# tan9zj/xnrs

Measured on AMD Instinct MI355X. Metric: impressions/sec (encode+score) on MIND-shaped batches, higher is better.
Workload: dtype f32; 1 GPU; NRMS full user+news encode + 5-candidate dot scoring (BASELINE configs[2]; token shape of config/mind_small_NRMS.yml); batch_impressions_per_gpu=512, history=50, candidates=5, d_backbone=768, n_heads=16, emb_dim=256, parallelism=impressions sharded by user over 1 GPU(s), no data-path collective

## Files before the change

### xnrs_amd/csrc/batch.hip

```cpp
#include <atomic>

#include "host.h"

namespace xnrs {

__device__ __forceinline__ uint64_t mix64(uint64_t seed, uint64_t a, uint64_t b) {
  uint64_t z = seed + 0x9E3779B97F4A7C15ull * (a * 0x100000001B3ull + b + 1);
  z = (z ^ (z >> 30)) * 0xBF58476D1CE4E5B9ull;
  z = (z ^ (z >> 27)) * 0x94D049BB133111EBull;
  return z ^ (z >> 31);
}

__global__ __launch_bounds__(256) void assemble_train_kernel(BatchArgs a) {
  const int64_t i = (int64_t)blockIdx.x * 256 + threadIdx.x;
  const int W = a.l_hist + 1 + a.n_neg;
  if (i >= a.B * W) return;
  const int64_t b = i / W;
  const int j = (int)(i - b * W);
  const int64_t s = a.sess[b];
  if (j < a.l_hist) {
    const int64_t lo = a.hist_off[s], hi = a.hist_off[s + 1];
    const int64_t n = (hi - lo < a.l_hist) ? (hi - lo) : a.l_hist;
    a.hist_out[b * a.l_hist + j] = (j < n) ? a.hist_val[hi - n + j] : a.pad_row;
  } else {
// ... 260 lines not shown
        w += __popcll(b);
        if (kept && sl < S) kv_src[e1 + sl] = (int32_t)(src0 + sl);
      }
      if (lane == 0) kv_block[j] = e1 / S;
    }
    __syncthreads();
  }
  bad = __syncthreads_or(bad);
  if (tid == 0) {
    counts[0] = s_carry[0];
    counts[1] = s_carry[1];
    counts[2] = bad ? 1 : 0;
  }
}

__global__ __launch_bounds__(1024) void compact_rows64_kernel(const float* __restrict__ mask, const int32_t* __restrict__ ids,
                                                               int64_t n_news, int64_t chunk, int S, int64_t* __restrict__ row_off_all,
                                                               int32_t* __restrict__ live_all, int32_t* __restrict__ kvs_all,
                                                               int32_t* __restrict__ kvb_all, int64_t* __restrict__ counts_all) {
  __shared__ unsigned long long s_bits[1024];
  __shared__ int64_t s_row[1024];
  __shared__ int s_ex[2][1024];
  __shared__ int s_wsum[2][16];
  __shared__ int s_carry[2];
  const int tid = threadIdx.x, wave = tid >> 6, lane = tid & 63;
  const int64_t news0 = (int64_t)blockIdx.x * chunk;
  const int cn = (int)(n_news - news0 < chunk ? n_news - news0 : chunk);
  int64_t* row_off = row_off_all + (int64_t)blockIdx.x * (chunk + 1);
  int32_t* live_src = live_all + (int64_t)blockIdx.x * chunk * S;
  int32_t* kv_src = kvs_all + (int64_t)blockIdx.x * chunk * S;
  int32_t* kv_block = kvb_all + (int64_t)blockIdx.x * chunk;
  int64_t* counts = counts_all + 3 * (int64_t)blockIdx.x;
  int bad = 0;
  if (tid < 2) s_carry[tid] = 0;
  if (tid == 0) row_off[0] = 0;
  for (int base = 0; base < cn; base += 1024) {
    const int nn = cn - base < 1024 ? cn - base : 1024;
    s_bits[tid] = 0ull;
    s_row[tid] = tid < nn ? (ids ? (int64_t)ids[news0 + base + tid] : news0 + base + tid) : 0;
    __syncthreads();
    const int n_el = nn * S;
    for (int i0 = tid; i0 < n_el; i0 += 4096) {
      float mv[4];
      int jj[4], sl[4];
#pragma unroll
      for (int u = 0; u < 4; ++u) {
        const int i = i0 + 1024 * u;
        jj[u] = (i < n_el ? i : 0) / S;
        sl[u] = (i < n_el ? i : 0) - jj[u] * S;
        mv[u] = i < n_el ? mask[s_row[jj[u]] * S + sl[u]] : 0.f;
// ... 13 lines not shown
      int x = v[which];
      for (int off = 1; off < 64; off <<= 1) {
        const int up = __shfl_up(x, off);
        if (lane >= off) x += up;
      }
      incl[which] = x;
      if (lane == 63) s_wsum[which][wave] = x;
    }
    __syncthreads();
    for (int which = 0; which < 2; ++which) {
      int before = s_carry[which];
      for (int w = 0; w < wave; ++w) before += s_wsum[which][w];
      s_ex[which][tid] = before + incl[which] - v[which];
    }
    if (tid < nn) {
      row_off[base + tid + 1] = s_ex[0][tid] + cnt;
      kv_block[base + tid] = s_ex[1][tid] / S;
    }
    __syncthreads();
    if (tid == 1023) {
      s_carry[0] = s_ex[0][1023] + v[0];
      s_carry[1] = s_ex[1][1023] + v[1];
    }
#pragma unroll 4
    for (int i = tid; i < n_el; i += 1024) {
      const int jj = i / S, sl = i - jj * S;
      const unsigned long long b = s_bits[jj];
      if (b == 0ull) continue;
      const int32_t src = (int32_t)(s_row[jj] * S + sl);
      kv_src[s_ex[1][jj] + sl] = src;
      if ((b >> sl) & 1ull) live_src[s_ex[0][jj] + __popcll(b & ((1ull << sl) - 1ull))] = src;
    }
    __syncthreads();
  }
  bad = __syncthreads_or(bad);
  if (tid == 0) {
    counts[0] = s_carry[0];
    counts[1] = s_carry[1];
    counts[2] = bad ? 1 : 0;
  }
}

__global__ __launch_bounds__(256) void row_counts_kernel(const float* __restrict__ mask, const int32_t* __restrict__ ids,
                                                          int64_t n_seq, int L, int32_t* __restrict__ cnt) {
  const int lane = threadIdx.x & 63;
  const int64_t seq = (int64_t)blockIdx.x * 4 + (threadIdx.x >> 6);
  if (seq >= n_seq) return;
  const float* mp = mask + (ids ? (int64_t)ids[seq] : seq) * L;
// ... 126 lines not shown
  return w;
}
void set_status_word(int32_t* w) {
  int dev = -1;
  (void)hipGetDevice(&dev);
  g_status_device.store(w ? dev : -1, std::memory_order_relaxed);
  g_status_word.store(w, std::memory_order_relaxed);
}

hipError_t launch_compact_rows(const float* mask, const int32_t* ids, int64_t n_news, int64_t chunk, int S, int64_t* row_off,
                               int32_t* live_src, int32_t* kv_src, int32_t* kv_block, int64_t* counts, hipStream_t stream) {
  if (n_news <= 0 || chunk <= 0) return hipSuccess;
  const int64_t passes = (n_news + chunk - 1) / chunk;
  if (passes > 0x7fffffffLL) return hipErrorInvalidValue;
  if (S <= 64)
    hipLaunchKernelGGL(compact_rows64_kernel, dim3((unsigned)passes), dim3(1024), 0, stream, mask, ids, n_news, chunk, S, row_off,
                       live_src, kv_src, kv_block, counts);
  else
    hipLaunchKernelGGL(compact_rows_kernel, dim3((unsigned)passes), dim3(1024), 0, stream, mask, ids, n_news, chunk, S, row_off,
                       live_src, kv_src, kv_block, counts);
  return hipGetLastError();
}

__global__ __launch_bounds__(1024) void live_tiles_kernel(const float* __restrict__ mask, const int32_t* __restrict__ ids,
                                                           int64_t n_seq, int64_t chunk, int L, int BM, int64_t cap,
                                                           uint8_t* __restrict__ alive_all, int64_t* __restrict__ n_tiles,
                                                           int32_t* __restrict__ tiles_all) {
  __shared__ int s_wsum[16];
  __shared__ int s_carry;
  const int tid = threadIdx.x, wave = tid >> 6, lane = tid & 63;
  const int64_t seq0 = (int64_t)blockIdx.x * chunk;
  const int64_t cn = n_seq - seq0 < chunk ? n_seq - seq0 : chunk;
  uint8_t* alive = alive_all + seq0;
  int32_t* tiles = tiles_all + (int64_t)blockIdx.x * cap;
  for (int64_t j = tid; j < cn; j += 1024) {
    const float* mp = mask + (ids ? (int64_t)ids[seq0 + j] : seq0 + j) * L;
    int any = 0;
#pragma unroll 4
    for (int s = 0; s < L; ++s) any |= mp[s] != 0.f ? 1 : 0;
    alive[j] = (uint8_t)any;
  }
  if (tid == 0) s_carry = 0;
  __syncthreads();
  const int64_t rows = cn * L;
  const int64_t nt = (rows + BM - 1) / BM;
  const uint64_t below = lane ? (~0ull >> (64 - lane)) : 0ull;
  for (int64_t base = 0; base < nt; base += 1024) {
    const int64_t t = base + tid;
    bool live = false;
    if (t < nt) {
      const int64_t r0 = t * BM, r1 = (r0 + BM < rows ? r0 + BM : rows) - 1;
      for (int64_t n = r0 / L; n <= r1 / L; ++n) live = live || alive[n] != 0;
    }
    const uint64_t b = __ballot(live);
    if (lane == 0) s_wsum[wave] = __popcll(b);
    __syncthreads();
    int before = s_carry;
    for (int w = 0; w < wave; ++w) before += s_wsum[w];
    if (live) tiles[before + __popcll(b & below)] = (int32_t)t;
    __syncthreads();
    if (tid == 0) {
      int tot = s_carry;
      for (int w = 0; w < 16; ++w) tot += s_wsum[w];
      s_carry = tot;
    }
    __syncthreads();
  }
  if (tid == 0) n_tiles[blockIdx.x] = s_carry;
}

hipError_t launch_live_tiles(const float* mask, const int32_t* ids, int64_t n_seq, int64_t chunk, int L, int BM, uint8_t* alive,
                             int64_t* n_tiles, int32_t* tiles, hipStream_t stream) {
  if (n_seq <= 0 || chunk <= 0 || L <= 0 || BM <= 0) return hipSuccess;
  const int64_t passes = (n_seq + chunk - 1) / chunk;
  const int64_t cap = live_tiles_cap(chunk, L, BM);
  if (passes > 0x7fffffffLL || cap > 0x7fffffffLL) return hipErrorInvalidValue;
  hipLaunchKernelGGL(live_tiles_kernel, dim3((unsigned)passes), dim3(1024), 0, stream, mask, ids, n_seq, chunk, L, BM, cap, alive,
                     n_tiles, tiles);
  return hipGetLastError();
}

}

using namespace xnrs;

extern "C" {

size_t xnrs_row_lists_workspace_bytes(int64_t n_seq) { return n_seq > 0 ? align_up((size_t)n_seq * sizeof(int32_t)) : 0; }

int32_t xnrs_build_row_lists(const float* m, const int32_t* ids, int64_t n_seq, int32_t L, int32_t* live_rows,
                             int32_t* live_src_rows, int32_t* kv_rows, int32_t* kv_src_rows, int64_t* counts, void* ws,
                             size_t ws_bytes, void* stream) {
  if (n_seq < 0 || L <= 0 || !m || !live_rows || !kv_rows || !counts) return XNRS_EINVAL;
// ... 60 lines not shown
```

### xnrs_amd/csrc/encoder_fwd.hip

```cpp
#include <vector>

#include "host.h"

using namespace xnrs;

namespace xnrs {

Plan make_plan(int64_t n_seq, int L, int D, int A, int E, bool att, bool additive, bool head, bool pooled, int64_t chunk,
               bool train, int n_heads) {
  Plan p{};
  if (train) chunk = n_seq > 0 ? n_seq : 1;
  if (chunk <= 0) chunk = 65536 / L;
  if (chunk > n_seq) chunk = n_seq;
  if (chunk < 1) chunk = 1;
  p.chunk = chunk;
  const size_t rows = (size_t)chunk * L;
  Carver c;
  p.off_qkv = c.take_if(att, rows * 3 * (size_t)D * F32);
  p.off_o = c.take_if(att, rows * (size_t)D * F32);
  p.off_y = c.take_if(att && pooled, rows * (size_t)D * F32);
  p.off_t = c.take_if(pooled && additive, rows * (size_t)A * F32);
  p.off_p = c.take_if(pooled && head, (size_t)n_seq * D * F32);
  p.off_h = c.take_if(pooled && head, (size_t)n_seq * E * F32);
  p.off_stats = c.take_if(train && att, (size_t)chunk * n_heads * L * 2 * F32);
// ... 3 lines not shown
  if (pooled && additive) pl += align_up(split_planes_bytes(A, D));
  p.off_planes = c.take(pl);
  NewsFusedPlan nf{};
  size_t nfb = 0;
  if (att && additive && !train) {
    if (n_heads <= 0) nfb = news_fused_img_bound_bytes(L, D, A);
    else if (news_fused_plan(L, D, n_heads, A, &nf)) nfb = nf.img_bytes;
  }
  p.off_nf = c.take_if(nfb != 0, nfb);
  p.off_nfo = c.take_if(nfb != 0, news_fused_scratch_bytes(L, D));
  const bool lt = att && pooled && !train;
  const size_t passes = (size_t)(((n_seq > 0 ? n_seq : 1) + chunk - 1) / chunk);
  p.off_lt_alive = c.take_if(lt, (size_t)(n_seq > 0 ? n_seq : 1));
  p.off_lt_n = c.take_if(lt, passes * sizeof(int64_t));
  p.off_lt_tiles = c.take_if(lt, passes * (size_t)live_tiles_cap(chunk, L, LIVE_TILE_BM) * sizeof(int32_t));
  p.fold = carve_fold(c, att && additive, n_seq, D, A);
  p.total = c.total();
  return p;
}

bool device_counts_ok(const float* x, int D, int A, const xnrs_mha_params* att, const xnrs_additive_params* pool) {
  auto al16 = [](const void* p) { return p == nullptr || (reinterpret_cast<uintptr_t>(p) & 15) == 0; };
  if (!knobs().gemm_buf || gemm_mode() != 0 || D % 4 != 0 || D < 4 || (A > 0 && A % 4 != 0)) return false;
  if (!al16(x) || (pool && !al16(pool->w1))) return false;
  if (att && !(al16(att->wq) && al16(att->wk) && al16(att->wv) && al16(att->wo))) return false;
  return (int64_t)D * D * 4 <= (1ll << 30) && (int64_t)A * D * 4 <= (1ll << 30);
}

}

// ... 282 lines not shown
  const bool lt = r.live_tiles && knobs().gemm_live_tiles && !train && pooled && m && att && !fused && !afused &&
                  n_seq * (int64_t)L >= knobs().gemm_live_tiles_min_rows &&
                  device_counts_ok(x, D, A, att, additive ? pool : nullptr);
  bool lt_qkv = false;
  if (lt && knobs().mha_skip_masked) {
    MhaCoreArgs probe = mha_core_args(qkv + D, 3 * (int64_t)D, att, o, p.chunk, L, D);
    probe.q = qkv;
    probe.mask = m;
    probe.skip_dead = 1;
    lt_qkv = mha_core_skips_dead(probe);
  }
  const bool lt_fc1 = lt && additive && rowdot;
  const int64_t lt_cap = live_tiles_cap(p.chunk, L, LIVE_TILE_BM);
  const int64_t* lt_n = at<int64_t>(w, p.off_lt_n);
  const int32_t* lt_tiles = at<int32_t>(w, p.off_lt_tiles);
  if (lt_qkv || lt_fc1)
    XNRS_TRY(launch_live_tiles(m, ids, n_seq, p.chunk, L, LIVE_TILE_BM, at<uint8_t>(w, p.off_lt_alive), at<int64_t>(w, p.off_lt_n),
                               at<int32_t>(w, p.off_lt_tiles), stream));
  std::vector<int64_t> lt_host;
  if ((lt_qkv && prof_on(0)) || (lt_fc1 && prof_on(3))) {
    lt_host.resize((size_t)((n_seq + p.chunk - 1) / p.chunk));
    if (hipStreamSynchronize(stream) != hipSuccess ||
        hipMemcpy(lt_host.data(), lt_n, lt_host.size() * sizeof(int64_t), hipMemcpyDeviceToHost) != hipSuccess)
      lt_host.clear();
  }
  for (int64_t c0 = 0; !fused && !afused && c0 < n_seq; c0 += p.chunk) {
    const int64_t nc = (n_seq - c0 < p.chunk) ? (n_seq - c0) : p.chunk;
    const int64_t rows = nc * L;
    const int64_t* ltn = lt_n + c0 / p.chunk;
    const int32_t* ltl = lt_tiles + (c0 / p.chunk) * lt_cap;
    const double lt_rows = (double)LIVE_TILE_BM *
                           (double)(lt_host.empty() ? (rows + LIVE_TILE_BM - 1) / LIVE_TILE_BM : lt_host[(size_t)(c0 / p.chunk)]);
    const int32_t* cids = ids ? ids + c0 : nullptr;
    const float* cx = ids ? x : x + c0 * (int64_t)L * D;
    const float* cm = m ? (ids ? m : m + c0 * (int64_t)L) : nullptr;

    const float* seq = cx;
    const int32_t* seq_ids = cids;
    if (att) {
      const int64_t ld3 = 3 * (int64_t)D;
      if (qkv_given) {
      } else if (live) {
        const double nl = (double)prof_count(0, cnt, 0, n_live, stream), nkv = (double)prof_count(0, cnt, 1, n_kv, stream);
        ProfScope ps(0, 2.0 * (kvl ? nkv : rows) * 2.0 * D * D + 2.0 * nl * (double)D * D, stream);
        GemmArgs g = qkv_projection(cx, {cids, L}, att, 1, qkv + D, ld3, rows, D, pqkv);
        if (kvl) {
          XNRS_TRY(launch_zero_dead_qkv(qkv, cm, cids, nc, L, D, stream));
// ... 5 lines not shown
          g.m_dev = cnt ? cnt + 1 : nullptr;
          g.m_fill_hint = 0.6f;
          if (n_kv > 0) XNRS_TRY(launch_gemm_f32(g, stream));
        } else {
          XNRS_TRY(launch_gemm_f32(g, stream));
          XNRS_TRY(launch_zero_cols(qkv, ld3, D, rows, stream));
        }
        if (n_live > 0) {
          GemmArgs q = gemm_linear(cx, {lvx, 1}, D, att->wq, att->bq, qkv, ld3, n_live, D, D, XNRS_ACT_NONE, pqkv[0]);
          q.c_scatter = 1;
          q.c_scatter_ids = live_rows;
          q.m_dev = cnt;
          q.m_fill_hint = 0.4f;
          XNRS_TRY(launch_gemm_f32(q, stream));
        }
      } else {
        GemmArgs g = qkv_projection(cx, {cids, L}, att, 0, qkv, ld3, rows, D, pqkv);
        if (lt_qkv) {
          g.live_n = ltn;
          g.live_tiles = ltl;
        }
        ProfScope ps(0, 2.0 * (lt_qkv ? lt_rows : (double)rows) * 3.0 * D * D, stream);
        XNRS_TRY(launch_gemm_f32(g, stream));
      }

      MhaCoreArgs ma = mha_core_args(qkv + D, ld3, att, o, nc, L, D);
      ma.q = qkv;
      ma.mask = cm;
      ma.mask_gather_ids = cids;
      ma.dropout_p = att->dropout_p;
// ... 31 lines not shown

    float* pooled_dst = (head ? pb : y) + c0 * (int64_t)D;
    float* hm_dst = hm ? hm + c0 : nullptr;
    if (additive) {
      if (live) {
        ProfScope ps(3, 2.0 * (double)prof_count(3, cnt, 0, n_live, stream) * (double)D * A, stream);
        XNRS_TRY(hipMemsetAsync(t, 0, (size_t)rows * A * sizeof(float), stream));
        if (n_live > 0) {
          GemmArgs fg = fc1_product(seq, {att ? live_rows : lvx, 1}, fc1, t, n_live, D, A, false, pool, p1);
          fg.c_scatter = 1;
          fg.c_scatter_ids = live_rows;
          fg.m_dev = cnt;
          fg.m_fill_hint = 0.4f;
          XNRS_TRY(launch_gemm_f32(fg, stream));
        }
      } else {
        GemmArgs fg = fc1_product(seq, {seq_ids, L}, fc1, t, rows, D, A, rowdot, pool, p1);
        if (lt_fc1) {
          fg.live_n = ltn;
          fg.live_tiles = ltl;
        }
        ProfScope ps(3, 2.0 * (lt_fc1 ? lt_rows : (double)rows) * (double)D * A, stream);
        XNRS_TRY(launch_gemm_f32(fg, stream));
      }
      AdditivePoolArgs pa = additive_pool_args(t, rowdot, pool, seq, nc, L, D, A);
      pa.skip_dead = lt_fc1 ? 1 : 0;
      pa.mask = cm;
      pa.mask_gather_ids = cids;
      pa.x_gather_ids = seq_ids;
      pa.y = fold ? pob + c0 * (int64_t)D : pooled_dst;
      pa.asum_out = fold ? asum + c0 : nullptr;
      pa.a_out = a_save ? a_save : (a_out ? a_out + c0 * (int64_t)L : nullptr);
      pa.hm_out = cm ? hm_dst : nullptr;
      {
        ProfScope ps(4, 2.0 * rows * (double)(A + D), stream);
        XNRS_TRY(launch_additive_pool(pa, stream));
      }
      if (a_save && a_out)
        XNRS_TRY(hipMemcpyAsync(a_out, a_save, (size_t)rows * sizeof(float), hipMemcpyDeviceToDevice, stream));
    } else {
      MeanPoolArgs mp{};
// ... 342 lines not shown
```

### xnrs_amd/csrc/gemm_f32.hip

```cpp
#include <atomic>
#include <cstdlib>
#include <type_traits>

#include "kernels.h"

namespace xnrs {

constexpr int KALIGN = 32;

__device__ __attribute__((aligned(16))) float g_zero_line[4] = {0.f, 0.f, 0.f, 0.f};

typedef unsigned u32x4 __attribute__((ext_vector_type(4)));
constexpr unsigned BUF_OOB = 0x40000000u;

template <int TM, int TN, bool A_COL, bool B_KN, bool VEC, int PIPE, int BK, bool BUF = false, int MINW = 2, bool GATH = false,
          int KG = 2, bool RDOT = false, bool MDEV = false, bool LIVE = false>
__global__ __launch_bounds__(256, MINW) void gemm_f32_kernel(const GemmArgs a, int m_tiles, int n_tiles_seg, int gn) {
  static_assert(!MDEV || (!A_COL && !B_KN), "device row counts: forward layout only");
  static_assert(!LIVE || (BUF && !MDEV), "live row tiles: buffer-load forward kernels, host row count");
  static_assert(!BUF || (!A_COL && !B_KN && VEC), "buffer loads are implemented for the forward layout");
  static_assert(!RDOT || PIPE == 5, "the fused row dots ride on the interleaved pipeline (its MFMA call is the swapped one)");
  static_assert(!GATH || BUF, "the gathered-A variant keeps buffer loads for B");
  constexpr int BM = 64 * TM, BN = 64 * TN;
  constexpr bool SWZ = BK == 16;
// ... 428 lines not shown
    static_assert(sizeof(float2) * BN <= sizeof(float) * A_SZ * NBUF, "bias / weight staging fits the A tile buffers");
    for (int c = tid; c < BN; c += 256) {
      const int col = n0 + c;
      const bool cok = col < a.Nseg;
      s_bw[c] = make_float2((bias && cok) ? bias[col] : 0.f, cok ? a.rowdot_w[col] : 0.f);
    }
    __syncthreads();
    const int half = lane >> 5;
    auto dots = [&](auto FAST) {
#pragma unroll
      for (int j = 0; j < TN; ++j) {
        const int cb = wn * 32 * TN + 32 * j;
#pragma unroll
        for (int i = 0; i < TM; ++i) {
          const float sc = rowdot_block_t_lds<decltype(FAST)::value>(acc[i][j], s_bw + cb, half);
          const int64_t row = m0 + wm * 32 * TM + 32 * i + (lane & 31);
          if (lane < 32 && row < Mrun && n0 + cb < a.Nseg) a.rowdot_out[row * a.ldrd + ((n0 + cb) >> 5)] = sc;
        }
      }
    };
    if (a.act == ACT_TANH_FAST) dots(std::true_type{});
    else dots(std::false_type{});
    return;
  }
  if constexpr (!A_COL) {
    if (a.c_scatter) {
      const int32_t* __restrict__ sids = a.c_scatter_ids ? a.c_scatter_ids : a.gather_ids;
      const bool one = a.gather_S == 1;
      float bvj[TN];
      int colj[TN];
#pragma unroll
      for (int j = 0; j < TN; ++j) {
// ... 319 lines not shown
  k.mha_pair = num("XNRS_MHA_PAIR", 1) != 0;
  k.mha_bwd_fused = num("XNRS_MHA_BWD_FUSED", 1) != 0;
  k.gemm_dw = (int)num("XNRS_GEMM_DW", 2);
  k.gemm_dw_tile = (int)num("XNRS_GEMM_DW_TILE", 256);
  k.fold_out = (int)num("XNRS_FOLD_OUT", 1);
  k.fc1_rowdot = num("XNRS_FC1_ROWDOT", 1) != 0;
  k.fold_train = (int)num("XNRS_FOLD_TRAIN", 1);
  k.news_fused = (int)num("XNRS_NEWS_FUSED", 1);
  k.news_fused_npw = (int)num("XNRS_NEWS_FUSED_NPW", 0);
  k.fast_tanh = num("XNRS_FAST_TANH", 1) != 0;
  k.additive_fused = (int)num("XNRS_ADDITIVE_FUSED", 1);
  k.af_fbuf = num("XNRS_AF_FBUF", 1) == 2 ? 2 : 1;
  k.mha_skip_masked = num("XNRS_MHA_SKIP_MASKED", 1) != 0;
  k.gemm_live_tiles = num("XNRS_GEMM_LIVE_TILES", 1) != 0;
  k.gemm_live_tiles_min_rows = num("XNRS_GEMM_LIVE_TILES_MIN_ROWS", 16384);
  k.bwd_side_stream = num("XNRS_BWD_SIDE_STREAM", 1) != 0;
  k.bwd_side_min_rows = num("XNRS_BWD_SIDE_MIN_ROWS", 0);
  k.gru_layout = num("XNRS_GRU_LAYOUT", 0) == 1 ? 1 : 0;
  const long long m = num("XNRS_GEMM_MODE", 0);
  k.gemm_mode_init = (m >= 0 && m <= 2) ? (int)m : 0;
  return k;
}
static Knobs g_knobs = read_knobs();
static std::atomic<int> g_gemm_mode{g_knobs.gemm_mode_init};
const Knobs& knobs() { return g_knobs; }
void reload_knobs() { g_knobs = read_knobs(); }
int gemm_mode() { return g_gemm_mode.load(std::memory_order_relaxed); }
void set_gemm_mode(int mode) { g_gemm_mode.store((mode >= 0 && mode <= 2) ? mode : 0, std::memory_order_relaxed); }

hipError_t launch_gemm_f32(const GemmArgs& a_in, hipStream_t stream, int* nsplit_used) {
// ... 19 lines not shown
  if (nsplit <= 1) {
    nsplit = 1;
    a.k_per_split = a.K > 0 ? a.K : 1;
  }
  if (nsplit_used) *nsplit_used = nsplit;
  a.nt_store = (!a.accumulate && !a.c_scatter && a.M * a.ldc * 4 >= (64ll << 20)) ? 1 : 0;
  if (a.colsum && !(a.a_col && a.b_kn)) return hipErrorInvalidValue;
  if (a.k_dev && !(a.a_col && a.b_kn)) return hipErrorInvalidValue;
  if (a.colsum_out && !a.colsum) return hipErrorInvalidValue;
  if (a.C2 && (nsplit <= 1 || !(a.a_col && a.b_kn) || a.c2_row0 <= 0 || a.c2_row0 >= a.M)) return hipErrorInvalidValue;
  bool cs_copy = false;
  if (a.colsum && a.colsum_out && nsplit == 1) {
    if (al16(a.colsum_out)) a.colsum = a.colsum_out;
    else cs_copy = true;
  }
  if (a.rowdot_out && (a.a_col || a.b_kn || a.nseg != 1 || nsplit != 1 || !a.rowdot_w || a.c_scatter || a.accumulate || a.aux_mode ||
                       (a.act != 2 && a.act != ACT_TANH_FAST)))
    return hipErrorInvalidValue;
  hipError_t e;
  const int mode = gemm_mode();
  const int64_t min_tiles = knobs().split_min_tiles;
  if (a.m_dev && (a.a_col || a.b_kn || nsplit != 1 || mode != 0)) return hipErrorInvalidValue;
  if (a.live_tiles && (a.a_col || a.b_kn || nsplit != 1 || mode != 0 || a.m_dev)) return hipErrorInvalidValue;
  if (a.rowscale && (a.a_col || a.b_kn || a.nseg != 1 || nsplit != 1 || !a.rowscale_vec || a.c_scatter || a.rowdot_out))
    return hipErrorInvalidValue;
  if (mode && !a.rowdot_out && !a.rowscale && !a.a_col && !a.b_kn && vec && nsplit == 1 &&
      ((a.M + 127) / 128) * ((a.Nseg + 127) / 128) * a.nseg >= min_tiles)
    return launch_gemm_split(a, mode == 1 ? 3 : 2, stream);
  if (!a.a_col && !a.b_kn) e = launch_layout<false, false>(a, vec, nsplit, stream);
  else if (!a.a_col && a.b_kn) e = launch_layout<false, true>(a, vec, nsplit, stream);
  else if (a.a_col && a.b_kn) {
    if (knobs().gemm_dw && gemm_dw_eligible(a)) e = launch_gemm_dw(a, nsplit, stream);
    else e = launch_layout<true, true>(a, vec, nsplit, stream);
// ... 18 lines not shown
```

### xnrs_amd/csrc/host.h

```cpp
#pragma once
#include <initializer_list>

#include "../../include/xnrs_hip.h"
#include "kernels.h"

namespace xnrs {

inline size_t align_up(size_t x, size_t a = 256) { return (x + a - 1) / a * a; }

inline int32_t hip_rc(hipError_t e) { return e == hipSuccess ? XNRS_OK : (int32_t)e; }

#define XNRS_TRY(expr)                       \
  do {                                       \
    hipError_t _e = (expr);                  \
    if (_e != hipSuccess) return hip_rc(_e); \
  } while (0)
#define XNRS_TRY_RC(expr)           \
  do {                              \
    int32_t _rc = (expr);           \
    if (_rc != XNRS_OK) return _rc; \
  } while (0)

struct Carver {
  size_t off = 0;
// ... 97 lines not shown
  f.fw = c.take_if(wanted, (size_t)A * D * F32);
  f.fb = c.take_if(wanted, (size_t)A * F32);
  f.po = c.take_if(wanted, (size_t)n_seq * D * F32);
  f.as = c.take_if(wanted, (size_t)n_seq * F32);
  f.fsl = c.take_if(wanted, (size_t)FOLD_SPLITS * A * D * F32);
  return f;
}

struct Plan {
  int64_t chunk;
  size_t off_qkv, off_o, off_y, off_t, off_p, off_h;
  size_t off_stats, off_a;
  size_t off_planes;
  size_t off_nf, off_nfo;
  size_t off_lt_alive, off_lt_n, off_lt_tiles;
  FoldRegions fold;
  size_t total;
};
Plan make_plan(int64_t n_seq, int L, int D, int A, int E, bool att, bool additive, bool head, bool pooled, int64_t chunk,
               bool train = false, int n_heads = 0);

struct SeqEncode {
  const float *x, *m;
  const int32_t* ids;
  int64_t n_seq;
  int L, D;
  const xnrs_mha_params* att;
  bool pooled;
  int pool_kind;
  const xnrs_additive_params* pool;
// ... 37 lines not shown
```

### xnrs_amd/csrc/kernels.h

```cpp
#pragma once
#include <hip/hip_runtime.h>
#include <stdint.h>

namespace xnrs {

typedef float f32x4 __attribute__((ext_vector_type(4)));
typedef float f32x16 __attribute__((ext_vector_type(16)));

struct Knobs {
  int gemm_pipe = 6;
  int gemm_bk = 32;
  int gemm_buf = 1;
  long long gemm_group = -1;
  int gemm_tile = -1;
  long long split_min_tiles = 512;
  bool fc1_rowdot = true;
  int fold_train = 1;
  int fold_out = 1;
  int gemm_dw = 2;
  int gemm_dw_tile = 256;
  int mha_lds = -1;
  bool mha_pair = true;
  int mha_headwave = 1;
  int mha_bwd_fused = 1;
  int news_fused = 1;
  int news_fused_npw = 0;
  int gemm_mode_init = 0;
  bool fast_tanh = true;
  int additive_fused = 1;
  int af_fbuf = 1;
  bool bwd_side_stream = true;
  long long bwd_side_min_rows = 0;
  bool gemm_live_tiles = true;
  long long gemm_live_tiles_min_rows = 16384;
  bool mha_skip_masked = true;
  int gru_layout = 0;
};
const Knobs& knobs();
void reload_knobs();

__device__ __forceinline__ int64_t load_dev_scalar(const int64_t* p) { return *p; }

struct GemmArgs {
  const float* A;
  int32_t a_col;
  const int32_t* gather_ids;
  int32_t gather_S;
  int32_t c_scatter;
  const int32_t* c_scatter_ids;
// ... 241 lines not shown
  const float* b2;
  const float* mask;
  const int32_t* mask_gather_ids;
  const int32_t* x_gather_ids;
  const float* x;
  int64_t ldx;
  float* y;
  float* a_out;
  float* hm_out;
  float* asum_out;
  int64_t n_seq;
  int32_t N, D, A;
  const int64_t* row_off;
  const int32_t* row_ids;
  int32_t skip_dead;
  const int64_t* poison;
};
hipError_t launch_additive_pool(const AdditivePoolArgs& a, hipStream_t stream);
hipError_t launch_fold_bias(const float* w1, const float* bo, const float* b1, float* bf, int A, int D, hipStream_t stream);
hipError_t launch_add_rowscaled_bias(float* p, int64_t ld, const float* s, const float* b, int64_t n, int D, hipStream_t stream);

struct MeanPoolArgs {
  const float* x;
  int64_t ldx;
  const float* mask;
  const int32_t* mask_gather_ids;
  const int32_t* x_gather_ids;
  float* y;
  float* hm_out;
  int64_t n_seq;
// ... 62 lines not shown
  float* targets_out;
};
hipError_t launch_gather_rows(const float* table, const int32_t* ids, float* out, int64_t n, int64_t row_floats,
                              hipStream_t stream);
hipError_t launch_poison(float* y, int64_t n, const int64_t* flags, int n_flags, int flag_stride, hipStream_t stream);
int32_t* status_word();
void set_status_word(int32_t* w);
hipError_t launch_compact_rows(const float* mask, const int32_t* ids, int64_t n_news, int64_t chunk, int S, int64_t* row_off,
                               int32_t* live_src, int32_t* kv_src, int32_t* kv_block, int64_t* counts, hipStream_t stream);
hipError_t launch_build_row_lists(const float* mask, const int32_t* ids, int64_t n_seq, int L, int32_t* live, int32_t* live_src,
                                  int32_t* kv, int32_t* kv_src, int64_t* counts, int32_t* cnt_scratch, hipStream_t stream);
constexpr int LIVE_TILE_BM = 128;
inline int64_t live_tiles_cap(int64_t chunk, int L, int BM) { return (chunk * L + BM - 1) / BM; }
hipError_t launch_live_tiles(const float* mask, const int32_t* ids, int64_t n_seq, int64_t chunk, int L, int BM, uint8_t* alive,
                             int64_t* n_tiles, int32_t* tiles, hipStream_t stream);
hipError_t launch_assemble_train(const BatchArgs& a, hipStream_t stream);
hipError_t launch_assemble_eval(const BatchArgs& a, hipStream_t stream);
hipError_t launch_score_csr(const float* vecs, const int32_t* rows, const int32_t* sess, const float* u, float* r, int64_t n,
                            int E, int relu, hipStream_t stream);
hipError_t launch_rank_metrics(const float* score, const float* target, const int64_t* off, float* out, int64_t B,
                               hipStream_t stream);

struct ColSumSeg {
  const float* X;
  int64_t ld;
  int64_t rows;
  int ncol;
  float* out;
};
hipError_t launch_colsum_segments(const ColSumSeg* segs, int n_segs, hipStream_t stream);
// ... 51 lines not shown
```

### xnrs_amd/csrc/mha_core.hip

```cpp
#include <cstdlib>

#include "kernels.h"

namespace xnrs {

template <int KT, bool VEC>
__global__ __launch_bounds__(256) void mha_core_kernel(MhaCoreArgs a, int QT, int64_t n_units) {
  const int lane = threadIdx.x & 63;
  const int64_t unit = (int64_t)blockIdx.x * 4 + (threadIdx.x >> 6);
  if (unit >= n_units) return;
  const int qt = (int)(unit % QT);
  const int64_t uh = unit / QT;
  const int hd = (int)(uh % a.n_heads);
  const int64_t seq = uh / a.n_heads;

  const int c = lane & 15, g = lane >> 4;
  const int S = a.S, dk = a.d_k;
  const int64_t row0 = seq * S;
  const int hoff = hd * dk;
  const int query = qt * 16 + c;
  const bool qvalid = query < S;

  f32x4 acc[KT];
#pragma unroll
// ... 448 lines not shown
          float* sp = a.stats + (((int64_t)seq * a.n_heads + hd) * (int64_t)S + query) * 2;
          sp[0] = -1e9f;
          sp[1] = (float)S;
        }
      }
      return;
    }
  }
  const bool tile_dead = a.skip_dead && a.mask && !a.q_off && !__any(qvalid && mq != 0.f);
  const float* qrow = a.q_off ? a.q + (q0 + (qvalid ? query : 0)) * a.ldq + hd * dk
                              : a.q + hbase + (int64_t)(qvalid ? query : 0) * ld;
  f32x4 qf[NFB];
#pragma unroll
  for (int fb = 0; fb < NFB; ++fb) {
    const int f0 = fb * 16 + 4 * g;
    qf[fb] = (qvalid && !tile_dead && f0 < dk) ? *reinterpret_cast<const f32x4*>(qrow + f0) : f32x4{0.f, 0.f, 0.f, 0.f};
  }

  {
    const int ch = tid % NCH, ks = tid / NCH;
    const int f0 = ch * 4, b = ch >> 2, g4 = ch & 3;
    const bool act = ks < KP;
    const bool fok = f0 < dk;
    const int vch = tid & 15, vkg = tid >> 4;
    const int vf0 = vch * 4, vb = vch >> 2, vg4 = vch & 3;
    const bool vact = vch < NCH && vkg < KTM * 4 + (TAIL ? 1 : 0);
    f32x4 kv[NPASS], vv[4];
#pragma unroll
    for (int ps = 0; ps < NPASS; ++ps) {
      const int key = ks + ps * KP;
      kv[ps] = f32x4{0.f, 0.f, 0.f, 0.f};
// ... 298 lines not shown
```

### xnrs_amd/csrc/pool_score.hip

```cpp
#include "host.h"

namespace xnrs {

__device__ __forceinline__ float wave_sum(float v) {
#pragma unroll
  for (int off = 32; off > 0; off >>= 1) v += __shfl_xor(v, off);
  return v;
}

constexpr int POOL_MAX_N = 512;

__global__ __launch_bounds__(256) void additive_pool_kernel(AdditivePoolArgs a) {
  __shared__ float s_w[POOL_MAX_N];
  __shared__ float s_red[4];
  __shared__ short s_idx[POOL_MAX_N];
  __shared__ int s_nlive;
  const int64_t seq = blockIdx.x;
  const int tid = threadIdx.x, lane = tid & 63, wave = tid >> 6;
  const int A = a.A, D = a.D;
  const int64_t src = a.mask_gather_ids ? (int64_t)a.mask_gather_ids[seq] : seq;
  const int64_t srcx = a.x_gather_ids ? (int64_t)a.x_gather_ids[seq] : seq;
  const bool csr = a.row_off != nullptr;
  const int64_t r0 = csr ? a.row_off[seq] : seq * a.N;
  const int N = csr ? (int)(a.row_off[seq + 1] - r0) : a.N;
// ... 5 lines not shown
    if (!__syncthreads_or(any)) {
      for (int d = tid; d < D; d += 256) a.y[seq * D + d] = 0.f;
      if (a.a_out)
        for (int i = tid; i < N; i += 256) a.a_out[r0 + i] = 0.f;
      if (tid == 0) {
        if (a.asum_out) a.asum_out[seq] = 0.f;
        if (a.hm_out) a.hm_out[seq] = 0.f;
      }
      return;
    }
  }

  const float b2 = a.b2 ? a.b2[0] : 0.f;
  if (a.epart) {
    for (int i = tid; i < N; i += 256) {
      const float* ep = a.epart + (r0 + i) * (int64_t)a.n_epart;
      float acc = 0.f;
      for (int s = 0; s < a.n_epart; ++s) acc += ep[s];
      float e = expf(acc + b2);
      if (mask) e *= mask[src * N + i];
      s_w[i] = e;
    }
  } else
  for (int i = wave; i < N; i += 4) {
    const float* t = a.t + (r0 + i) * (int64_t)A;
    float acc = 0.f;
    for (int k = lane; k < A; k += 64) acc = fmaf(t[k], a.w2[k], acc);
    acc = wave_sum(acc);
    if (lane == 0) {
      float e = expf(acc + b2);
// ... 223 lines not shown
```

Before: 18140 impressions/s.

## Compute Q and FC1 projections only on live (unmasked) token rows via gathered GEMM

Adds a dense row-list pass that fuses row compaction and live-tile listing into one kernel. It produces per-chunk lists of unmasked token positions. The Q projection and the additive-attention FC1 GEMM then gather only live rows and scatter results back, with rowdot output support for scatter added. Masked rows are skipped in pooling and zeroed in MHA query loads, so leftover garbage in unwritten rows is never used. This cuts GEMM FLOPs on padded tokens at the cost of gather/scatter indirection and a device-side row count.

```diff
diff --git a/xnrs_amd/csrc/batch.hip b/xnrs_amd/csrc/batch.hip
--- a/xnrs_amd/csrc/batch.hip
+++ b/xnrs_amd/csrc/batch.hip
@@ -298,10 +298,23 @@
   }
 }
 
+struct DenseLists {
+  int32_t* live_loc;
+  uint8_t* alive;
+  int64_t* n_tiles;
+  int32_t* tiles;
+  int64_t cap;
+  int BM;
+};
+__device__ void list_live_tiles(const uint8_t* __restrict__ alive, int64_t cn, int L, int BM, int32_t* __restrict__ tiles,
+                                int64_t* __restrict__ n_out, int* s_wsum, int* s_carry);
+
+template <bool DENSE>
 __global__ __launch_bounds__(1024) void compact_rows64_kernel(const float* __restrict__ mask, const int32_t* __restrict__ ids,
                                                                int64_t n_news, int64_t chunk, int S, int64_t* __restrict__ row_off_all,
                                                                int32_t* __restrict__ live_all, int32_t* __restrict__ kvs_all,
-                                                               int32_t* __restrict__ kvb_all, int64_t* __restrict__ counts_all) {
+                                                               int32_t* __restrict__ kvb_all, int64_t* __restrict__ counts_all,
+                                                               DenseLists dl) {
   __shared__ unsigned long long s_bits[1024];
   __shared__ int64_t s_row[1024];
   __shared__ int s_ex[2][1024];
@@ -310,14 +323,16 @@
   const int tid = threadIdx.x, wave = tid >> 6, lane = tid & 63;
   const int64_t news0 = (int64_t)blockIdx.x * chunk;
   const int cn = (int)(n_news - news0 < chunk ? n_news - news0 : chunk);
-  int64_t* row_off = row_off_all + (int64_t)blockIdx.x * (chunk + 1);
-  int32_t* live_src = live_all + (int64_t)blockIdx.x * chunk * S;
-  int32_t* kv_src = kvs_all + (int64_t)blockIdx.x * chunk * S;
-  int32_t* kv_block = kvb_all + (int64_t)blockIdx.x * chunk;
+  int64_t* row_off = DENSE ? nullptr : row_off_all + (int64_t)blockIdx.x * (chunk + 1);
+  int32_t* live_src = live_all ? live_all + (int64_t)blockIdx.x * chunk * S : nullptr;
+  int32_t* kv_src = DENSE ? nullptr : kvs_all + (int64_t)blockIdx.x * chunk * S;
+  int32_t* kv_block = DENSE ? nullptr : kvb_all + (int64_t)blockIdx.x * chunk;
   int64_t* counts = counts_all + 3 * (int64_t)blockIdx.x;
+  int32_t* live_loc = DENSE ? dl.live_loc + (int64_t)blockIdx.x * chunk * S : nullptr;
+  uint8_t* alive = DENSE ? dl.alive + news0 : nullptr;
   int bad = 0;
   if (tid < 2) s_carry[tid] = 0;
-  if (tid == 0) row_off[0] = 0;
+  if (!DENSE && tid == 0) row_off[0] = 0;
   for (int base = 0; base < cn; base += 1024) {
     const int nn = cn - base < 1024 ? cn - base : 1024;
     s_bits[tid] = 0ull;
@@ -361,8 +376,12 @@
       s_ex[which][tid] = before + incl[which] - v[which];
     }
     if (tid < nn) {
-      row_off[base + tid + 1] = s_ex[0][tid] + cnt;
-      kv_block[base + tid] = s_ex[1][tid] / S;
+      if constexpr (DENSE) {
+        alive[base + tid] = bits != 0ull ? 1 : 0;
+      } else {
+        row_off[base + tid + 1] = s_ex[0][tid] + cnt;
+        kv_block[base + tid] = s_ex[1][tid] / S;
+      }
     }
     __syncthreads();
     if (tid == 1023) {
@@ -375,10 +394,28 @@
       const unsigned long long b = s_bits[jj];
       if (b == 0ull) continue;
       const int32_t src = (int32_t)(s_row[jj] * S + sl);
-      kv_src[s_ex[1][jj] + sl] = src;
-      if ((b >> sl) & 1ull) live_src[s_ex[0][jj] + __popcll(b & ((1ull << sl) - 1ull))] = src;
-    }
-    __syncthreads();
+      if constexpr (DENSE) {
+        if ((b >> sl) & 1ull) {
+          const int at = s_ex[0][jj] + __popcll(b & ((1ull << sl) - 1ull));
+          live_loc[at] = (int32_t)((base + jj) * S + sl);
+          if (live_src) live_src[at] = src;
+        }
+      } else {
+        kv_src[s_ex[1][jj] + sl] = src;
+        if ((b >> sl) & 1ull) live_src[s_ex[0][jj] + __popcll(b & ((1ull << sl) - 1ull))] = src;
+      }
+    }
+    __syncthreads();
+  }
+  if constexpr (DENSE) {
+    if (tid == 0) {
+      counts[0] = s_carry[0];
+      counts[1] = s_carry[1];
+      s_carry[0] = 0;
+    }
+    __syncthreads();
+    list_live_tiles(alive, cn, S, dl.BM, dl.tiles + (int64_t)blockIdx.x * dl.cap, dl.n_tiles + blockIdx.x, s_wsum[0], &s_carry[0]);
+    return;
   }
   bad = __syncthreads_or(bad);
   if (tid == 0) {
@@ -535,8 +572,8 @@
   const int64_t passes = (n_news + chunk - 1) / chunk;
   if (passes > 0x7fffffffLL) return hipErrorInvalidValue;
   if (S <= 64)
-    hipLaunchKernelGGL(compact_rows64_kernel, dim3((unsigned)passes), dim3(1024), 0, stream, mask, ids, n_news, chunk, S, row_off,
-                       live_src, kv_src, kv_block, counts);
+    hipLaunchKernelGGL(compact_rows64_kernel<false>, dim3((unsigned)passes), dim3(1024), 0, stream, mask, ids, n_news, chunk, S,
+                       row_off, live_src, kv_src, kv_block, counts, DenseLists{});
   else
     hipLaunchKernelGGL(compact_rows_kernel, dim3((unsigned)passes), dim3(1024), 0, stream, mask, ids, n_news, chunk, S, row_off,
                        live_src, kv_src, kv_block, counts);
@@ -549,7 +586,7 @@
                                                            int32_t* __restrict__ tiles_all) {
   __shared__ int s_wsum[16];
   __shared__ int s_carry;
-  const int tid = threadIdx.x, wave = tid >> 6, lane = tid & 63;
+  const int tid = threadIdx.x;
   const int64_t seq0 = (int64_t)blockIdx.x * chunk;
   const int64_t cn = n_seq - seq0 < chunk ? n_seq - seq0 : chunk;
   uint8_t* alive = alive_all + seq0;
@@ -563,6 +600,12 @@
   }
   if (tid == 0) s_carry = 0;
   __syncthreads();
+  list_live_tiles(alive, cn, L, BM, tiles, n_tiles + blockIdx.x, s_wsum, &s_carry);
+}
+
+__device__ void list_live_tiles(const uint8_t* __restrict__ alive, int64_t cn, int L, int BM, int32_t* __restrict__ tiles,
+                                int64_t* __restrict__ n_out, int* s_wsum, int* s_carry) {
+  const int tid = threadIdx.x, wave = tid >> 6, lane = tid & 63;
   const int64_t rows = cn * L;
   const int64_t nt = (rows + BM - 1) / BM;
   const uint64_t below = lane ? (~0ull >> (64 - lane)) : 0ull;
@@ -576,18 +619,18 @@
     const uint64_t b = __ballot(live);
     if (lane == 0) s_wsum[wave] = __popcll(b);
     __syncthreads();
-    int before = s_carry;
+    int before = *s_carry;
     for (int w = 0; w < wave; ++w) before += s_wsum[w];
     if (live) tiles[before + __popcll(b & below)] = (int32_t)t;
     __syncthreads();
     if (tid == 0) {
-      int tot = s_carry;
+      int tot = *s_carry;
       for (int w = 0; w < 16; ++w) tot += s_wsum[w];
-      s_carry = tot;
-    }
-    __syncthreads();
-  }
-  if (tid == 0) n_tiles[blockIdx.x] = s_carry;
+      *s_carry = tot;
+    }
+    __syncthreads();
+  }
+  if (tid == 0) *n_out = *s_carry;
 }
 
 hipError_t launch_live_tiles(const float* mask, const int32_t* ids, int64_t n_seq, int64_t chunk, int L, int BM, uint8_t* alive,
@@ -598,6 +641,18 @@
   if (passes > 0x7fffffffLL || cap > 0x7fffffffLL) return hipErrorInvalidValue;
   hipLaunchKernelGGL(live_tiles_kernel, dim3((unsigned)passes), dim3(1024), 0, stream, mask, ids, n_seq, chunk, L, BM, cap, alive,
                      n_tiles, tiles);
+  return hipGetLastError();
+}
+
+hipError_t launch_dense_row_lists(const float* mask, const int32_t* ids, int64_t n_seq, int64_t chunk, int L, int BM,
+                                  int32_t* live_loc, int32_t* live_src, int64_t* counts, uint8_t* alive, int64_t* n_tiles,
+                                  int32_t* tiles, hipStream_t stream) {
+  if (n_seq <= 0 || chunk <= 0 || L <= 0 || BM <= 0) return hipSuccess;
+  const int64_t passes = (n_seq + chunk - 1) / chunk;
+  const int64_t cap = live_tiles_cap(chunk, L, BM);
+  if (L > 64 || passes > 0x7fffffffLL || cap > 0x7fffffffLL || chunk * L > 0x7fffffffLL) return hipErrorInvalidValue;
+  hipLaunchKernelGGL(compact_rows64_kernel<true>, dim3((unsigned)passes), dim3(1024), 0, stream, mask, ids, n_seq, chunk, L,
+                     nullptr, ids ? live_src : nullptr, nullptr, nullptr, counts, DenseLists{live_loc, alive, n_tiles, tiles, cap, BM});
   return hipGetLastError();
 }
 
diff --git a/xnrs_amd/csrc/encoder_fwd.hip b/xnrs_amd/csrc/encoder_fwd.hip
--- a/xnrs_amd/csrc/encoder_fwd.hip
+++ b/xnrs_amd/csrc/encoder_fwd.hip
@@ -41,6 +41,10 @@
   p.off_lt_alive = c.take_if(lt, (size_t)(n_seq > 0 ? n_seq : 1));
   p.off_lt_n = c.take_if(lt, passes * sizeof(int64_t));
   p.off_lt_tiles = c.take_if(lt, passes * (size_t)live_tiles_cap(chunk, L, LIVE_TILE_BM) * sizeof(int32_t));
+  const bool lr = lt && L <= 64;
+  p.off_lr_loc = c.take_if(lr, passes * rows * sizeof(int32_t));
+  p.off_lr_src = c.take_if(lr, passes * rows * sizeof(int32_t));
+  p.off_lr_cnt = c.take_if(lr, passes * 3 * sizeof(int64_t));
   p.fold = carve_fold(c, att && additive, n_seq, D, A);
   p.total = c.total();
   return p;
@@ -353,15 +357,30 @@
   const int64_t lt_cap = live_tiles_cap(p.chunk, L, LIVE_TILE_BM);
   const int64_t* lt_n = at<int64_t>(w, p.off_lt_n);
   const int32_t* lt_tiles = at<int32_t>(w, p.off_lt_tiles);
-  if (lt_qkv || lt_fc1)
+  const bool lr = lt && knobs().gemm_live_rows && p.off_lr_cnt != 0 && L <= 64 && n_seq * (int64_t)L <= 0x7fffffffLL &&
+                  n_seq * (int64_t)L >= knobs().gemm_live_rows_min_rows;
+  const bool lr_qkv = lr && lt_qkv, lr_fc1 = lr && lt_fc1;
+  const int32_t *lr_loc = at<int32_t>(w, p.off_lr_loc), *lr_src = at<int32_t>(w, p.off_lr_src);
+  const int64_t* lr_cnt = at<int64_t>(w, p.off_lr_cnt);
+  constexpr float LR_FILL = 0.3f;
+  if (lr_qkv || lr_fc1)
+    XNRS_TRY(launch_dense_row_lists(m, ids, n_seq, p.chunk, L, LIVE_TILE_BM, at<int32_t>(w, p.off_lr_loc), at<int32_t>(w, p.off_lr_src),
+                                    at<int64_t>(w, p.off_lr_cnt), at<uint8_t>(w, p.off_lt_alive), at<int64_t>(w, p.off_lt_n),
+                                    at<int32_t>(w, p.off_lt_tiles), stream));
+  else if (lt_qkv || lt_fc1)
     XNRS_TRY(launch_live_tiles(m, ids, n_seq, p.chunk, L, LIVE_TILE_BM, at<uint8_t>(w, p.off_lt_alive), at<int64_t>(w, p.off_lt_n),
                                at<int32_t>(w, p.off_lt_tiles), stream));
-  std::vector<int64_t> lt_host;
+  std::vector<int64_t> lt_host, lr_host;
   if ((lt_qkv && prof_on(0)) || (lt_fc1 && prof_on(3))) {
     lt_host.resize((size_t)((n_seq + p.chunk - 1) / p.chunk));
     if (hipStreamSynchronize(stream) != hipSuccess ||
         hipMemcpy(lt_host.data(), lt_n, lt_host.size() * sizeof(int64_t), hipMemcpyDeviceToHost) != hipSuccess)
       lt_host.clear();
+    if (lr_qkv || lr_fc1) {
+      lr_host.resize(3 * lt_host.size());
+      if (lt_host.empty() || hipMemcpy(lr_host.data(), lr_cnt, lr_host.size() * sizeof(int64_t), hipMemcpyDeviceToHost) != hipSuccess)
+        lr_host.clear();
+    }
   }
   for (int64_t c0 = 0; !fused && !afused && c0 < n_seq; c0 += p.chunk) {
     const int64_t nc = (n_seq - c0 < p.chunk) ? (n_seq - c0) : p.chunk;
@@ -370,6 +389,10 @@
     const int32_t* ltl = lt_tiles + (c0 / p.chunk) * lt_cap;
     const double lt_rows = (double)LIVE_TILE_BM *
                            (double)(lt_host.empty() ? (rows + LIVE_TILE_BM - 1) / LIVE_TILE_BM : lt_host[(size_t)(c0 / p.chunk)]);
+    const int32_t* lrl = lr_loc + (c0 / p.chunk) * p.chunk * L;
+    const int32_t* lrs = lr_src + (c0 / p.chunk) * p.chunk * L;
+    const int64_t* lrn = lr_cnt + 3 * (c0 / p.chunk);
+    const double lr_rows = lr_host.empty() ? (double)rows : (double)lr_host[(size_t)(3 * (c0 / p.chunk))];
     const int32_t* cids = ids ? ids + c0 : nullptr;
     const float* cx = ids ? x : x + c0 * (int64_t)L * D;
     const float* cm = m ? (ids ? m : m + c0 * (int64_t)L) : nullptr;
@@ -405,6 +428,18 @@
           q.m_fill_hint = 0.4f;
           XNRS_TRY(launch_gemm_f32(q, stream));
         }
+      } else if (lr_qkv) {
+        ProfScope ps(0, 2.0 * lt_rows * 2.0 * D * D + 2.0 * lr_rows * (double)D * D, stream);
+        GemmArgs g = qkv_projection(cx, {cids, L}, att, 1, qkv + D, ld3, rows, D, pqkv);
+        g.live_n = ltn;
+        g.live_tiles = ltl;
+        XNRS_TRY(launch_gemm_f32(g, stream));
+        GemmArgs q = gemm_linear(cx, {ids ? lrs : lrl, 1}, D, att->wq, att->bq, qkv, ld3, rows, D, D);
+        q.c_scatter = 1;
+        q.c_scatter_ids = lrl;
+        q.m_dev = lrn;
+        q.m_fill_hint = LR_FILL;
+        XNRS_TRY(launch_gemm_f32(q, stream));
       } else {
         GemmArgs g = qkv_projection(cx, {cids, L}, att, 0, qkv, ld3, rows, D, pqkv);
         if (lt_qkv) {
@@ -466,6 +501,14 @@
           fg.m_fill_hint = 0.4f;
           XNRS_TRY(launch_gemm_f32(fg, stream));
         }
+      } else if (lr_fc1) {
+        GemmArgs fg = fc1_product(seq, {seq_ids ? lrs : lrl, 1}, fc1, t, rows, D, A, true, pool, p1);
+        fg.c_scatter = 1;
+        fg.c_scatter_ids = lrl;
+        fg.m_dev = lrn;
+        fg.m_fill_hint = LR_FILL;
+        ProfScope ps(3, 2.0 * lr_rows * (double)D * A, stream);
+        XNRS_TRY(launch_gemm_f32(fg, stream));
       } else {
         GemmArgs fg = fc1_product(seq, {seq_ids, L}, fc1, t, rows, D, A, rowdot, pool, p1);
         if (lt_fc1) {
@@ -477,6 +520,7 @@
       }
       AdditivePoolArgs pa = additive_pool_args(t, rowdot, pool, seq, nc, L, D, A);
       pa.skip_dead = lt_fc1 ? 1 : 0;
+      pa.skip_masked = lr_fc1 ? 1 : 0;
       pa.mask = cm;
       pa.mask_gather_ids = cids;
       pa.x_gather_ids = seq_ids;
diff --git a/xnrs_amd/csrc/gemm_f32.hip b/xnrs_amd/csrc/gemm_f32.hip
--- a/xnrs_amd/csrc/gemm_f32.hip
+++ b/xnrs_amd/csrc/gemm_f32.hip
@@ -466,8 +466,13 @@
 #pragma unroll
         for (int i = 0; i < TM; ++i) {
           const float sc = rowdot_block_t_lds<decltype(FAST)::value>(acc[i][j], s_bw + cb, half);
-          const int64_t row = m0 + wm * 32 * TM + 32 * i + (lane & 31);
-          if (lane < 32 && row < Mrun && n0 + cb < a.Nseg) a.rowdot_out[row * a.ldrd + ((n0 + cb) >> 5)] = sc;
+          int64_t row = m0 + wm * 32 * TM + 32 * i + (lane & 31);
+          if (lane < 32 && row < Mrun && n0 + cb < a.Nseg) {
+            if constexpr (GATH && MDEV) {
+              if (a.c_scatter) row = (a.c_scatter_ids ? a.c_scatter_ids : a.gather_ids)[row];
+            }
+            a.rowdot_out[row * a.ldrd + ((n0 + cb) >> 5)] = sc;
+          }
         }
       }
     };
@@ -817,6 +822,8 @@
   k.mha_skip_masked = num("XNRS_MHA_SKIP_MASKED", 1) != 0;
   k.gemm_live_tiles = num("XNRS_GEMM_LIVE_TILES", 1) != 0;
   k.gemm_live_tiles_min_rows = num("XNRS_GEMM_LIVE_TILES_MIN_ROWS", 16384);
+  k.gemm_live_rows = num("XNRS_GEMM_LIVE_ROWS", 1) != 0;
+  k.gemm_live_rows_min_rows = num("XNRS_GEMM_LIVE_ROWS_MIN_ROWS", 16384);
   k.bwd_side_stream = num("XNRS_BWD_SIDE_STREAM", 1) != 0;
   k.bwd_side_min_rows = num("XNRS_BWD_SIDE_MIN_ROWS", 0);
   k.gru_layout = num("XNRS_GRU_LAYOUT", 0) == 1 ? 1 : 0;
@@ -866,9 +873,10 @@
     if (al16(a.colsum_out)) a.colsum = a.colsum_out;
     else cs_copy = true;
   }
-  if (a.rowdot_out && (a.a_col || a.b_kn || a.nseg != 1 || nsplit != 1 || !a.rowdot_w || a.c_scatter || a.accumulate || a.aux_mode ||
+  if (a.rowdot_out && (a.a_col || a.b_kn || a.nseg != 1 || nsplit != 1 || !a.rowdot_w || a.accumulate || a.aux_mode ||
                        (a.act != 2 && a.act != ACT_TANH_FAST)))
     return hipErrorInvalidValue;
+  if (a.rowdot_out && a.c_scatter && !(a.gather_ids && a.gather_S == 1 && a.m_dev)) return hipErrorInvalidValue;
   hipError_t e;
   const int mode = gemm_mode();
   const int64_t min_tiles = knobs().split_min_tiles;
diff --git a/xnrs_amd/csrc/host.h b/xnrs_amd/csrc/host.h
--- a/xnrs_amd/csrc/host.h
+++ b/xnrs_amd/csrc/host.h
@@ -135,6 +135,7 @@
   size_t off_planes;
   size_t off_nf, off_nfo;
   size_t off_lt_alive, off_lt_n, off_lt_tiles;
+  size_t off_lr_loc, off_lr_src, off_lr_cnt;
   FoldRegions fold;
   size_t total;
 };
diff --git a/xnrs_amd/csrc/kernels.h b/xnrs_amd/csrc/kernels.h
--- a/xnrs_amd/csrc/kernels.h
+++ b/xnrs_amd/csrc/kernels.h
@@ -33,6 +33,8 @@
   long long bwd_side_min_rows = 0;
   bool gemm_live_tiles = true;
   long long gemm_live_tiles_min_rows = 16384;
+  bool gemm_live_rows = true;
+  long long gemm_live_rows_min_rows = 16384;
   bool mha_skip_masked = true;
   int gru_layout = 0;
 };
@@ -304,6 +306,7 @@
   const int64_t* row_off;
   const int32_t* row_ids;
   int32_t skip_dead;
+  int32_t skip_masked;
   const int64_t* poison;
 };
 hipError_t launch_additive_pool(const AdditivePoolArgs& a, hipStream_t stream);
@@ -396,6 +399,9 @@
 inline int64_t live_tiles_cap(int64_t chunk, int L, int BM) { return (chunk * L + BM - 1) / BM; }
 hipError_t launch_live_tiles(const float* mask, const int32_t* ids, int64_t n_seq, int64_t chunk, int L, int BM, uint8_t* alive,
                              int64_t* n_tiles, int32_t* tiles, hipStream_t stream);
+hipError_t launch_dense_row_lists(const float* mask, const int32_t* ids, int64_t n_seq, int64_t chunk, int L, int BM,
+                                  int32_t* live_loc, int32_t* live_src, int64_t* counts, uint8_t* alive, int64_t* n_tiles,
+                                  int32_t* tiles, hipStream_t stream);
 hipError_t launch_assemble_train(const BatchArgs& a, hipStream_t stream);
 hipError_t launch_assemble_eval(const BatchArgs& a, hipStream_t stream);
 hipError_t launch_score_csr(const float* vecs, const int32_t* rows, const int32_t* sess, const float* u, float* r, int64_t n,
diff --git a/xnrs_amd/csrc/mha_core.hip b/xnrs_amd/csrc/mha_core.hip
--- a/xnrs_amd/csrc/mha_core.hip
+++ b/xnrs_amd/csrc/mha_core.hip
@@ -486,7 +486,7 @@
 #pragma unroll
   for (int fb = 0; fb < NFB; ++fb) {
     const int f0 = fb * 16 + 4 * g;
-    qf[fb] = (qvalid && !tile_dead && f0 < dk) ? *reinterpret_cast<const f32x4*>(qrow + f0) : f32x4{0.f, 0.f, 0.f, 0.f};
+    qf[fb] = (qvalid && !tile_dead && mq != 0.f && f0 < dk) ? *reinterpret_cast<const f32x4*>(qrow + f0) : f32x4{0.f, 0.f, 0.f, 0.f};
   }
 
   {
diff --git a/xnrs_amd/csrc/pool_score.hip b/xnrs_amd/csrc/pool_score.hip
--- a/xnrs_amd/csrc/pool_score.hip
+++ b/xnrs_amd/csrc/pool_score.hip
@@ -43,6 +43,13 @@
   const float b2 = a.b2 ? a.b2[0] : 0.f;
   if (a.epart) {
     for (int i = tid; i < N; i += 256) {
+      if (a.skip_masked && mask) {
+        const float mi = mask[src * N + i];
+        if (mi == 0.f) {
+          s_w[i] = mi;
+          continue;
+        }
+      }
       const float* ep = a.epart + (r0 + i) * (int64_t)a.n_epart;
       float acc = 0.f;
       for (int s = 0; s < a.n_epart; ++s) acc += ep[s];
```

Result: faster. 20630 impressions/s, median of 6 (+13.8%).
